# thomasantony/splat

Hardware: AMD Instinct MI355X
Metric: frames_per_sec (higher is better)
Workload: dtype f32

## Files before the change

### splat_amd/csrc/splat_api.hip

```cpp
#include <algorithm>
#include <cmath>
#include <cstdio>
#include <cstdlib>
#include <cstring>
#include <mutex>
#include <new>
#include <string>
#include <unordered_map>
#include <vector>

#include "splat_context.h"

using namespace splat;

static thread_local std::string g_create_error;
static std::mutex g_ledger_mu;
static std::unordered_map<void*, std::pair<splat_ctx*, size_t>> g_ledger;

namespace splat {
CommState** ctx_comm_slot(splat_ctx* c) { return &c->comm; }
hipStream_t ctx_stream(splat_ctx* c) { return c->stream; }
hipStream_t frame_stream(splat_ctx* c) { return (c->last_lane && c->comp2) ? c->comp2 : c->stream; }
int frame_tail(splat_ctx* c) {
    if (c->last_ring < 0 || !c->ring[c->last_ring].used) return SPLAT_OK;
// ... 145 lines not shown

int ensure_lane(splat_ctx* c) {
    if (c->comp2 || c->pipeline == 0) return SPLAT_OK;
    HIP_TRY(c, ensure_copy_stream(c));
    c->comp2 = c->copy_stream;
    return SPLAT_OK;
}

SceneArgs scene_of(const splat_ctx* c) { return {c->n, c->planes, c->orig, c->bounds}; }
HintTable hint_table(const splat_ctx* c, size_t stride) { return {c->need_hint, stride}; }
HintTable hint_table(const splat_ctx* c) { return hint_table(c, c->m_alloc); }

int ensure_bins(splat_ctx* c, unsigned int m) {
    if (m + 1 <= c->m_alloc) return SPLAT_OK;
    int rc = sync_all(c);
    if (rc != SPLAT_OK) return rc;
    c->m_alloc = 0;
    bump_epoch(c);
    c->sort_hint = false;
    dfree(c->zero_layout);
    HIP_TRY(c, dmalloc(c, &c->zero_layout, sizeof(unsigned int) * (size_t)(m + 1)));
    HIP_TRY(c, fill_now(c->zero_layout, 0, sizeof(unsigned int) * (size_t)(m + 1)));
    dfree(c->need_hint);
    HIP_TRY(c, dmalloc(c, &c->need_hint, hint_table(c, (size_t)(m + 1)).bytes()));
    HIP_TRY(c, fill_now(c->need_hint, 0, hint_table(c, (size_t)(m + 1)).bytes()));
    for (Slot& s : c->slots) {
        dfree(s.counts); dfree(s.offsets); dfree(s.cursor); dfree(s.order); dfree(s.lens); dfree(s.counts_b); dfree(s.lay_a); dfree(s.lay_b);
        dfree(s.near_m); dfree(s.redo_layout); dfree(s.redo_cursors); dfree(s.off2);
        s.layout_valid = false; s.flip = 0;
        HIP_TRY(c, dmalloc(c, &s.off2, sizeof(unsigned int) * (size_t)(m + 1)));
        HIP_TRY(c, dmalloc(c, &s.near_m, sizeof(unsigned int) * (size_t)(m + 1)));
        HIP_TRY(c, dmalloc(c, &s.redo_layout, sizeof(unsigned int) * (size_t)(m + 1)));
        HIP_TRY(c, dmalloc(c, &s.redo_cursors, sizeof(unsigned int) * (size_t)(m + 1)));
        HIP_TRY(c, dmalloc(c, &s.counts_b, sizeof(unsigned int) * (size_t)(m + 1)));
        HIP_TRY(c, dmalloc(c, &s.lay_a, sizeof(unsigned int) * (size_t)(m + 1)));
        HIP_TRY(c, dmalloc(c, &s.lay_b, sizeof(unsigned int) * (size_t)(m + 1)));
        HIP_TRY(c, dmalloc(c, &s.lens, sizeof(unsigned int) * (size_t)(m + 1)));
        HIP_TRY(c, dmalloc(c, &s.counts, sizeof(unsigned int) * (size_t)(m + 1)));
        HIP_TRY(c, dmalloc(c, &s.offsets, sizeof(unsigned int) * (size_t)(m + 1)));
        HIP_TRY(c, dmalloc(c, &s.cursor, sizeof(unsigned int) * (size_t)(m + 1)));
        HIP_TRY(c, dmalloc(c, &s.order, sizeof(unsigned int) * (size_t)(m + 1)));
        HIP_TRY(c, fill_now(s.counts, 0, sizeof(unsigned int) * (size_t)(m + 1)));
    }
    c->m_alloc = m + 1;
    return SPLAT_OK;
}
// ... 305 lines not shown
    c->iters_valid = false;
    if (want_iters) {
        if (c->iters_alloc < m * 4u) {
            dfree(c->d_iters); c->iters_alloc = 0;
            HIP_TRY(c, dmalloc(c, &c->d_iters, sizeof(uint2) * (size_t)m * 4u));
            c->iters_alloc = m * 4u;
        }
        HIP_TRY(c, hipMemsetAsync(c->d_iters, 0, sizeof(uint2) * (size_t)m * 4u, cs));
        iters = c->d_iters;
        c->iters_valid = true;
    }
    CompositeArgs comp{};
    comp.s = cs; comp.knobs = &c->knobs; comp.n_tiles = m; comp.fc = c->fc; comp.recs = s.recs; comp.argb = d_argb; comp.status = f.d_st; comp.orig = c->orig;
    comp.fused_sort_max = retained ? 0u : c->fused_sort_max; comp.iters = iters; comp.keep_keys = want_iters || f.retain == SPLAT_RETAIN_WRITER;
    comp.pair_walk = pd.pair_walk != 0;
    comp.libm_exp = (c->cfg.mode & SPLAT_MODE_LIBM_EXP) != 0; comp.clear_first = c->clear_first;
    comp.lists = f.lists; comp.lists.near_m = pd.near_cap ? s.near_m : nullptr;
    comp.keys = f.keys; comp.keys.keys2 = pd.comp_sorts != 0 ? s.keys2 : nullptr;
    if (retained) {
        const bool near = c->ret_set.near_cap != 0u;
        comp.lists.near_m = near ? s.near_m : nullptr; comp.keys.keys2 = near ? s.keys2 : nullptr;
    }
    comp.hints = hint_table(c);
    comp.refine = c->fc.close_width == 0.0f ? pd.refine : 0u;
    launch_composite(comp);
    c->last_near = retained ? c->ret_set.near_cap != 0u : pd.near_cap != 0u;
    HIP_TRY(c, f.mark(6, cs));
    if (want_iters) HIP_TRY(c, hipMemcpyAsync(&c->h_status[f.r], f.d_st, sizeof(FrameStatus), hipMemcpyDeviceToHost, cs));
    HIP_TRY(c, hipEventRecord(f.ev->e[7], cs));
    return SPLAT_OK;
}

int decide_retention(splat_ctx* c, const splat_camera* cam, int* action) {
    splat_retain_input in;
    std::memset(&in, 0, sizeof in);
    static_assert(sizeof(splat_camera) + 2 * sizeof(int32_t) <= sizeof in.cam, "the camera and the slab fit the decision's words");
    std::memcpy(in.cam, cam, sizeof(splat_camera));
    const int32_t slab[2] = {c->slab0, c->slab1};
    std::memcpy(reinterpret_cast<unsigned char*>(in.cam) + sizeof(splat_camera), slab, sizeof slab);
    in.epoch = c->bin_epoch; in.still_frames = c->pol.still_frames;
    in.enabled = (c->retain_lists != 0 && c->knobs.dbg_ntiles == 0u) ? 1 : 0;
    in.overlap = c->overlap; in.one_pass = c->fc.bucket_cap ? 1 : 0;
    splat_retain_decision d;
    const int wr = c->ret_set.ring;
    for (int pass = 0; pass < 2; ++pass) {
        if (c->ret.writer == 1u && wr >= 0) {
// ... 427 lines not shown
        c->env_pinned |= 1u << SPLAT_OPT_NEAR_SELECT_KEYS;
    }
    option_from_env(c, SPLAT_OPT_HOST_ZERO_COPY, "SPLAT_HOST_ZERO_COPY", 0, 1);
    option_from_env(c, SPLAT_OPT_COUNT_FIRST, "SPLAT_COUNT_FIRST", 0, 2);
    if (const char* kg = std::getenv("SPLAT_KEYS_PER_GAUSSIAN")) {
        const int v = std::atoi(kg);
        c->keys_per_gaussian = v <= 0 ? 0u : (unsigned int)std::min(256, std::max(4, v));
        c->env_pinned |= 1u << SPLAT_OPT_KEYS_PER_GAUSSIAN;
    }
    option_from_env(c, SPLAT_OPT_LARGE_SPLAT_TILES, "SPLAT_LARGE_TILES", -1, 1048576);
    option_from_env(c, SPLAT_OPT_LARGE_LIST_MIN, "SPLAT_LARGE_LIST_MIN", -1, 1e9);
    option_from_env(c, SPLAT_OPT_START_REFINE, "SPLAT_START_REFINE", 0, 1);
    option_from_env(c, SPLAT_OPT_RETAIN_LISTS, "SPLAT_RETAIN", 0, 1);
    if (const char* lm = std::getenv("SPLAT_LAYOUT_MOTION")) c->layout_motion = std::atoi(lm) != 0 ? 1 : 0;
    if (const char* k1 = std::getenv("SPLAT_SORT_RADIX_MIN")) c->knobs.sort_radix_min = (unsigned int)std::max(0, std::atoi(k1));
    if (const char* k2 = std::getenv("SPLAT_SCAN_THREADS")) c->knobs.scan_threads = std::atoi(k2);
    if (const char* k3 = std::getenv("SPLAT_DBG_NTILES")) c->knobs.dbg_ntiles = (unsigned int)std::max(0, std::atoi(k3));
    if (const char* k8 = std::getenv("SPLAT_DBG_SELECT_STRIDE")) c->knobs.dbg_select_stride = (unsigned int)std::max(0, std::atoi(k8));
    if (const char* k10 = std::getenv("SPLAT_START_HINTS")) { c->start_hints = std::min(2, std::max(0, std::atoi(k10))); c->env_pinned |= 1u << SPLAT_OPT_START_HINTS; }
    if (const char* k7 = std::getenv("SPLAT_DBG_ONE_PASS_SELECT")) c->one_pass_select = std::atoi(k7) != 0;
    if (const char* k11 = std::getenv("SPLAT_DBG_KEYS2_ENTRIES")) c->knobs.dbg_keys2_entries = std::strtoull(k11, nullptr, 10);
    if (const char* k9 = std::getenv("SPLAT_DBG_HINT_RADIUS")) c->knobs.dbg_hint_radius = std::atoi(k9);
    if (const char* k12 = std::getenv("SPLAT_DBG_SELECT_BLIND")) c->knobs.dbg_select_blind = std::atoi(k12) != 0 ? 1u : 0u;
    if (const char* k5 = std::getenv("SPLAT_DBG_STARTS")) c->knobs.dbg_starts = std::atoi(k5) != 0 ? 1u : 0u;
    if (const char* k4 = std::getenv("SPLAT_COMP_LDS_PAD")) c->knobs.comp_lds_pad = (unsigned int)std::max(0, std::atoi(k4));
    if (const char* k1p = std::getenv("SPLAT_K1_LDS_PAD")) c->knobs.k1_lds_pad = (unsigned int)std::min(48 * 1024, std::max(0, std::atoi(k1p)));
    auto bail = [&](const char* what, hipError_t err) {
        g_create_error = std::string(what) + ": " + hipGetErrorString(err);
        splat_destroy(c);
        return SPLAT_ERR_HIP;
    };
    if ((e = hipSetDevice(cfg->device)) != hipSuccess) return bail("hipSetDevice", e);
    if ((e = init_device_kernels()) != hipSuccess) return bail("hipFuncSetAttribute", e);
    if ((e = hipStreamCreateWithFlags(&c->stream, hipStreamNonBlocking)) != hipSuccess) return bail("hipStreamCreate", e);
    c->own_stream = true;
    {
        int lo = 0, hi = 0;
        (void)hipDeviceGetStreamPriorityRange(&lo, &hi);
        int prio = c->pipeline >= 6 ? (lo + hi) / 2 : hi;
        if (const char* ep = std::getenv("SPLAT_BIN_PRIO")) prio = std::atoi(ep) > 0 ? hi : (std::atoi(ep) < 0 ? lo : (lo + hi) / 2);
        if ((e = hipStreamCreateWithPriority(&c->bin_stream, hipStreamNonBlocking, prio)) != hipSuccess) return bail("hipStreamCreate", e);
        if ((e = hipStreamCreateWithPriority(&c->sort_stream, hipStreamNonBlocking, prio)) != hipSuccess) return bail("hipStreamCreate", e);
    }
    if (c->overlap >= 2 && c->pipeline) { if ((e = ensure_copy_stream(c)) != hipSuccess) return bail("hipStreamCreate", e); c->comp2 = c->copy_stream; }
    for (Slot& s : c->slots) {
        if ((e = dmalloc(c, &s.d_status, sizeof(FrameStatus))) != hipSuccess) return bail("hipMalloc(status)", e);
// ... 1 lines not shown
        if ((e = hipEventCreateWithFlags(&s.ev_ready, hipEventDisableTiming)) != hipSuccess) return bail("hipEventCreate", e);
        if ((e = hipEventCreateWithFlags(&s.ev_binned, hipEventDisableTiming)) != hipSuccess) return bail("hipEventCreate", e);
    }
    if ((e = dmalloc(c, &c->d_status_ring, sizeof(FrameStatus) * EV_RING)) != hipSuccess) return bail("hipMalloc(status ring)", e);
    if ((e = fill_now(c->d_status_ring, 0, sizeof(FrameStatus) * EV_RING)) != hipSuccess) return bail("fill_now(status ring)", e);
    if ((e = hipHostMalloc(&c->h_status, sizeof(FrameStatus) * EV_RING, hipHostMallocCoherent)) != hipSuccess) return bail("hipHostMalloc(status)", e);
    std::memset(c->h_status, 0, sizeof(FrameStatus) * EV_RING);
    for (auto& s : c->ring)
        for (auto& ev : s.e)
            if ((e = hipEventCreate(&ev)) != hipSuccess) return bail("hipEventCreate", e);
    *out = c;
    return SPLAT_OK;
}

void splat_destroy(splat_ctx* c) {
    if (!c) return;
    (void)hipSetDevice(c->cfg.device);
    if (c->bin_stream) (void)hipStreamSynchronize(c->bin_stream);
    if (c->sort_stream) (void)hipStreamSynchronize(c->sort_stream);
    if (c->stream) (void)hipStreamSynchronize(c->stream);
    if (c->copy_stream) (void)hipStreamSynchronize(c->copy_stream);
    if (c->comm) { comm_release(c->comm); c->comm = nullptr; }
    free_scene(c);
    dfree(c->zero_layout); dfree(c->need_hint);
    for (Slot& s : c->slots) {
        dfree(s.counts); dfree(s.offsets); dfree(s.cursor); dfree(s.order); dfree(s.lens); dfree(s.counts_b); dfree(s.lay_a); dfree(s.lay_b);
        dfree(s.near_m); dfree(s.redo_layout); dfree(s.redo_cursors); dfree(s.off2);
        dfree(s.keys); dfree(s.keys2); dfree(s.d_status);
        if (s.ev_ready) (void)hipEventDestroy(s.ev_ready);
        if (s.ev_binned) (void)hipEventDestroy(s.ev_binned);
    }
    dfree(c->d_img); dfree(c->d_iters);
    for (int k = 0; k < splat_ctx::S_IMGS; ++k) {
        dfree(c->s_img[k]);
        if (c->s_rendered[k]) (void)hipEventDestroy(c->s_rendered[k]);
        if (c->s_copied[k]) (void)hipEventDestroy(c->s_copied[k]);
    }
    if (c->copy_stream) { (void)hipStreamSynchronize(c->copy_stream); (void)hipStreamDestroy(c->copy_stream); }
    if (c->h_status) (void)hipHostFree(c->h_status);
    dfree(c->d_status_ring);
    for (auto& s : c->ring)
        for (auto& ev : s.e)
            if (ev) (void)hipEventDestroy(ev);
    if (c->bin_stream) (void)hipStreamDestroy(c->bin_stream);
    if (c->sort_stream) (void)hipStreamDestroy(c->sort_stream);
    if (c->own_stream && c->stream) (void)hipStreamDestroy(c->stream);
    {
// ... 573 lines not shown
```

### splat_amd/csrc/splat_context.h

```cpp
#ifndef SPLAT_CONTEXT_H
#define SPLAT_CONTEXT_H
#include <string>
#include <vector>

#include "splat_internal.h"
#include "../../include/splat_policy.h"
#include "../../include/splat_retain.h"

#define HIP_TRY(ctx, expr)                                                                             \
    do {                                                                                               \
        hipError_t _e = (expr);                                                                        \
        if (_e != hipSuccess) {                                                                        \
            (ctx)->err = std::string(#expr) + ": " + hipGetErrorString(_e);                            \
            return SPLAT_ERR_HIP;                                                                      \
        }                                                                                              \
    } while (0)

namespace splat {
constexpr int N_EV = 9;
constexpr int N_TIMES = 6;
constexpr int EV_RING = 32;
static_assert(EV_RING == SPLAT_POLICY_RING, "the frame policy sees the whole status ring");
constexpr int N_SLOTS = 4;

// ... 88 lines not shown
    uint64_t cap = 0;
    uint64_t cap2 = 0;
    uint64_t keys2_want = 0;
    bool use_buckets = true;
    bool bucket_failed = false;
    uint64_t bucket_bytes = 128ull << 30;
    uint64_t layout_want = 0;
    unsigned int layout_m = 0;
    bool last_one_pass = false;
    unsigned int* zero_layout = nullptr;
    uint64_t dev_bytes = 0, dev_bytes_peak = 0;
    splat::LaunchKnobs knobs;
    float region_spare = 4.0f;
    uint64_t frame_idx = 0;
    uint64_t bin_idx = 0;
    int retain_lists = 1;
    uint64_t bin_epoch = 0;
    splat_retain_state ret{};
    uint64_t frames_retained = 0;
    struct RetainSet {
        int slot = -1, ring = -1;
        unsigned int near_cap = 0;
        splat::FrameStatus status{};
    } ret_set;
    int last_slot = -1;
    bool last_lists_in_memory = false;
    splat::FrameStatus* h_status = nullptr;
    splat::FrameStatus* d_status_ring = nullptr;
    bool clear_first = false;
    uint32_t* d_img = nullptr;
    size_t img_cap = 0;
    static constexpr int S_IMGS = 4;
    uint32_t* s_img[S_IMGS] = {};
    size_t s_cap = 0;
    hipStream_t copy_stream = nullptr;
    hipEvent_t s_rendered[S_IMGS] = {}, s_copied[S_IMGS] = {};
    const uint32_t* s_dst[S_IMGS] = {};
    bool s_used[S_IMGS] = {};
    uint64_t s_idx = 0;
    int s_ring[S_IMGS] = {-1, -1, -1, -1};
    splat_camera s_cam[S_IMGS] = {};
    int slab0 = 0, slab1 = -1;
    splat::EvSet ring[splat::EV_RING];
    int ring_next = 0;
    int last_ring = -1;
    double acc_ms[splat::N_TIMES] = {0, 0, 0, 0, 0, 0};
    uint64_t acc_frames = 0;
// ... 58 lines not shown
```

### splat_amd/csrc/splat_internal.h

```cpp
#ifndef SPLAT_INTERNAL_H
#define SPLAT_INTERNAL_H
#include <hip/hip_runtime.h>
#include <stdint.h>

#include "../../include/splat_hip.h"

#ifndef SPLAT_K1X
#define SPLAT_K1X 0
#endif
#ifndef SPLAT_EXP_STAGE2
#define SPLAT_EXP_STAGE2 0
#endif
#ifndef SPLAT_EXP_K1DUMMY
#define SPLAT_EXP_K1DUMMY 0
#endif
#ifndef SPLAT_EXP_SKIPFULL
#define SPLAT_EXP_SKIPFULL 0
#endif
#ifndef SPLAT_EXP_SORT2
#define SPLAT_EXP_SORT2 0
#endif
#ifndef SPLAT_EXP_K1DROP
#define SPLAT_EXP_K1DROP 0
#endif
// ... 56 lines not shown
    unsigned int n_probe_fail;
    unsigned int pad_;
    unsigned long long n_blocks_culled;
    unsigned long long layout_total;
};

struct Rec {
    float4 a;
    float4 b;
    float4 c;
};

struct LaunchKnobs {
    unsigned int sort_radix_min = 128;
    int scan_threads = 0;
    unsigned int dbg_ntiles = 0;
    unsigned int comp_lds_pad = 0;
    unsigned int k1_lds_pad = 0;
    unsigned int dbg_select_stride = 0;
    unsigned long long dbg_keys2_entries = 0;
    int dbg_hint_radius = -1;
    unsigned int dbg_select_blind = 0;
    unsigned int dbg_starts = 0;
};

struct HintTable {
    unsigned int* base;
    size_t stride;

    static constexpr unsigned int NEED_PLANE = 0u, NEED_PLANES = 4u;
    static constexpr unsigned int DEPTH_PLANE = NEED_PLANE + NEED_PLANES, DEPTH_PLANES = 1u;
    static constexpr unsigned int START_PLANE = DEPTH_PLANE + DEPTH_PLANES, START_PLANES = 4u;
    static constexpr unsigned int REFINE_PLANE = START_PLANE + START_PLANES, REFINE_PLANES = 4u;
    static constexpr unsigned int HINT_WORDS = 13u;
    static_assert(DEPTH_PLANE == 4u && START_PLANE == 5u && REFINE_PLANE == 9u && REFINE_PLANE + REFINE_PLANES == HINT_WORDS,
                  "the four parts tile the table exactly");

    unsigned int* plane(unsigned int k) const { return base ? base + k * stride : nullptr; }
    unsigned int* needs() const { return plane(NEED_PLANE); }
    unsigned int* select_depth() const { return plane(DEPTH_PLANE); }
    unsigned int* starts() const { return plane(START_PLANE); }
    unsigned int* refinement() const { return plane(REFINE_PLANE); }
    size_t words() const { return HINT_WORDS * stride; }
    size_t bytes() const { return sizeof(unsigned int) * words(); }
};

// ... 125 lines not shown
    unsigned int near_cap;
    const unsigned int* need_hint;
    unsigned int* near_thr;
    unsigned int tiles_x, tile_rows;
    unsigned int grid;
    bool at_rest;
    int hint_radius;
};
void launch_select(const SelectArgs& a);

struct CompositeArgs {
    hipStream_t s; const LaunchKnobs* knobs; unsigned int n_tiles; FrameConst fc;
    TileLists lists;
    KeyBuffers keys;
    const Rec* recs; uint32_t* argb; FrameStatus* status; const unsigned int* orig;
    unsigned int fused_sort_max;
    uint2* iters;
    bool keep_keys;
    bool pair_walk;
    bool libm_exp;
    bool clear_first;
    HintTable hints;
    unsigned int refine;
};
void launch_composite(const CompositeArgs& a);
void launch_status_set(hipStream_t s, FrameStatus* status, const FrameStatus& v);
hipError_t init_device_kernels();

struct CommState;
CommState** ctx_comm_slot(splat_ctx* c);
hipStream_t ctx_stream(splat_ctx* c);
hipStream_t frame_stream(splat_ctx* c);
int ctx_device(const splat_ctx* c);
int frame_tail(splat_ctx* c);
int ctx_quiesce(splat_ctx* c);
int ctx_fail(splat_ctx* c, int code, const char* msg);
void comm_release(CommState* s);

}
#endif
```

### splat_amd/csrc/splat_kernels.hip

```cpp
#include <algorithm>
#include <cstddef>
#include <cstdlib>
#include <type_traits>

#include "splat_internal.h"
#include "splat_device_math.h"

namespace splat {
static constexpr unsigned long long KERNELS_EXP2F_TAB[32] = {
    0x3ff0000000000000ull, 0x3fefd9b0d3158574ull, 0x3fefb5586cf9890full, 0x3fef9301d0125b51ull, 0x3fef72b83c7d517bull,
    0x3fef54873168b9aaull, 0x3fef387a6e756238ull, 0x3fef1e9df51fdee1ull, 0x3fef06fe0a31b715ull, 0x3feef1a7373aa9cbull,
    0x3feedea64c123422ull, 0x3feece086061892dull, 0x3feebfdad5362a27ull, 0x3feeb42b569d4f82ull, 0x3feeab07dd485429ull,
    0x3feea47eb03a5585ull, 0x3feea09e667f3bcdull, 0x3fee9f75e8ec5f74ull, 0x3feea11473eb0187ull, 0x3feea589994cce13ull,
    0x3feeace5422aa0dbull, 0x3feeb737b0cdc5e5ull, 0x3feec49182a3f090ull, 0x3feed503b23e255dull, 0x3feee89f995ad3adull,
    0x3feeff76f2fb5e47ull, 0x3fef199bdd85529cull, 0x3fef3720dcef9069ull, 0x3fef5818dcfba487ull, 0x3fef7c97337b9b5full,
    0x3fefa4afa2a490daull, 0x3fefd0765b6e4540ull};
constexpr bool exp2f_tab_is_the_headers() {
    for (int i = 0; i < 32; ++i) if (KERNELS_EXP2F_TAB[i] != EXP2F_TAB_HOST[i]) return false;
    return true;
}
static_assert(exp2f_tab_is_the_headers(), "splat_kernels.hip's copy of EXP2F_TAB differs from splat_device_math.h's");
}


// ... 2254 lines not shown
           (unsigned long long)(unsigned int)__builtin_amdgcn_readfirstlane((int)(unsigned int)v);
}

struct WaveLds { float4 a[64]; float4 b[64]; float4 c[64]; };

#ifndef SPLAT_REFINE_MIN_STEP
#define SPLAT_REFINE_MIN_STEP 8
#endif
#ifndef SPLAT_COMP_WAVES
#define SPLAT_COMP_WAVES 1
#endif
struct CompArgs {
    FrameConst fc;
    const unsigned int* offsets; const unsigned int* order; const unsigned int* lens;
    unsigned long long* keys; const Rec* recs; uint32_t* argb; FrameStatus* status;
    unsigned int fused_sort_max, radix_min;
    uint2* iters;
    unsigned int keep_keys, clear_first;
    const unsigned int* orig;
    unsigned long long* keys2; const unsigned int* near_m;
    unsigned int* need_hint; unsigned int* start_hint; const unsigned int* off2;
    unsigned int* probe_hint;
    unsigned int refine;
};
typedef const __attribute__((address_space(4))) CompArgs* KernArgs;
template <bool PAIR, bool LIBM>
static __device__ void repair_tile(KernArgs ka, unsigned int smem_lds, unsigned int exptab_lds, unsigned int item, bool again);

template <bool PAIR, bool LIBM, int LONGM>
__device__ __forceinline__ void composite_tile(unsigned char* smem, const unsigned long long* exptab, const unsigned int item, const FrameConst& fc,
                                               const unsigned int* __restrict__ offsets, const unsigned int* __restrict__ order,
                                               const unsigned int* __restrict__ lens, unsigned long long* __restrict__ keys,
                                               const Rec* __restrict__ recs, uint32_t* __restrict__ argb,
                                               FrameStatus* __restrict__ status, unsigned int fused_sort_max,
                                               unsigned int radix_min, uint2* __restrict__ iters, unsigned int keep_keys,
                                               const unsigned int* __restrict__ orig, const unsigned int clear_first,
                                               unsigned long long* __restrict__ keys2, const unsigned int* __restrict__ near_m,
                                               unsigned int* __restrict__ need_hint, unsigned int* __restrict__ start_hint,
                                               const unsigned int* __restrict__ off2, KernArgs ka ,
                                               const bool walk_this_wave = true, const bool second_walk = false ) {
    auto late = [&]() -> KernArgs {
        unsigned long long p = (unsigned long long)(size_t)ka;
        asm volatile("" : "+s"(p));
        return (KernArgs)(size_t)p;
    };
    static_assert(sizeof(WaveLds) * 4 <= sort_lds_bytes<256, 2048>(), "staging fits the sort workspace");
    WaveLds* slds = reinterpret_cast<WaveLds*>(smem);
    const unsigned int tile = (unsigned int)__builtin_amdgcn_readfirstlane((int)order[item]);
    const unsigned int tid = threadIdx.x;
    const unsigned int beg = __builtin_amdgcn_readfirstlane(offsets[tile]);
    const unsigned int end = beg + __builtin_amdgcn_readfirstlane(lens[tile]);
    if (beg == end) {
// ... 121 lines not shown
            } else {
                L.a[slot] = r.a; L.b[slot] = r.b;
                L.c[slot] = make_float4(r.c.x, r.c.y, r.c.z, __uint_as_float(base + lane));
            }
        }
        const unsigned int kk = (unsigned int)__builtin_popcountll(m);
        if (pair_layout && (kk & 1u) && lane == 0) {
            float* P = reinterpret_cast<float*>(&L) + (kk >> 1) * 24u + 1u;
            P[0] = 0.0f; P[2] = 0.0f; P[4] = -1.0f; P[6] = -1.0f; P[8] = 0.0f; P[10] = 0.0f; P[12] = 0.0f; P[14] = 0.0f;
            float* Q = reinterpret_cast<float*>(&L) + (kk >> 1) * 24u + 2u;
            Q[16] = 0.0f; Q[17] = 0.0f; Q[20] = 0.0f;
        }
        __builtin_amdgcn_fence(__ATOMIC_ACQUIRE, "wavefront");
        __builtin_amdgcn_wave_barrier();
        return kk;
    };
    auto expv = [&](float x) -> float {
        if constexpr (LIBM) return exp_libm(x, exptab);
        else return exp_neg(x);
    };

    bool need_far = false;
    unsigned int itA = 0, itB = 0;
    float alast = -1.0f;
    if (!need_far) {
        bool found = !inside;
        Rec r;
        unsigned int cntN = min(64u, end - lb), bsN = end - cntN;
        fetch(bsN, cntN, r);
        while (true) {
            const unsigned int bs = bsN, cnt = cntN;
            const unsigned int k = stage(r, cnt, bs, false);
            if (bs > lb) { cntN = min(64u, bs - lb); bsN = bs - cntN; fetch(bsN, cntN, r); }
            unsigned int jsel = 0xffffffffu;
            for (unsigned int j = k; j-- > 0;) {
                const float4 a = L.a[j];
                const bool cov = (fabsf(sxm - a.x) <= a.z) & (fabsf(a.y - sym) <= a.w);
                jsel = (cov & !found) ? j : jsel;
                found = found | cov;
                if (__builtin_amdgcn_ballot_w64(!found) == 0ull) break;
            }
            if (__builtin_amdgcn_ballot_w64(jsel != 0xffffffffu) != 0ull) {
                const unsigned int jr = (jsel != 0xffffffffu) ? jsel : 0u;
                const float4 a = L.a[jr], b = L.b[jr];
                bool cov;
                const float alpha = fragment_alpha(sxm, sym, a, b, expv, cov);
// ... 41 lines not shown
            const unsigned int k = stage(r, cnt, bs, true, true, false, -1, 0u, nA < 32u ? (int)nA : -1);
            nA += nA < 32u ? 1u : 0u;
            if (bs > lb) { cntN = min(64u, bs - lb); bsN = bs - cntN; fetch(bsN, cntN, r); }
            for (unsigned int j = k; j-- > 0;) {
                const float4 a = L.a[j], b = L.b[j];
                const float dx = sxm - a.x, dy = a.y - sym;
                const float p2 = fmaf(dx, fmaf(b.x, dx, b.y * dy), (b.z * dy) * dy) + b.w;
                float alpha = fminf(0.99f, __builtin_amdgcn_exp2f(p2));
                alpha = (p2 < -7.994353f) ? 0.0f : alpha;
                T = fmaf(-alpha, T, T);
                const bool now = !done & (T < fc.early_eps);
                sp = now ? __float_as_uint(a.z) : sp;
                done = done | now;
            }
            itA += k;
            if (__builtin_amdgcn_ballot_w64(!done) == 0ull || bs == lb || bs <= giveup) break;
        }
        unsigned int need = done ? sp : lb;
#pragma unroll
        for (int o = 32; o > 0; o >>= 1) need = min(need, (unsigned int)__shfl_xor((int)need, o));
        ws = (unsigned int)__builtin_amdgcn_readfirstlane((int)need);
        if (ws == 0xffffffffu) ws = end;
    }

    const float cw = fc.close_width;
    float R = (float)((old >> 16) & 0xffu), G = (float)((old >> 8) & 0xffu), B = (float)(old & 0xffu);
    float R2 = 255.0f, G2 = 255.0f, B2 = 255.0f;
    auto shade = [&](auto BRt, const float4& a, const float4& b, const float4& c) {
        constexpr bool BR = decltype(BRt)::value;
        bool cov;
        const float alpha = fragment_alpha(sxm, sym, a, b, expv, cov);
        const float ia = 1.0f - alpha;
        const float ar = alpha * c.x, ag = alpha * c.y, ab = alpha * c.z;
        R = blend_channel(R, ia, ar);
        G = blend_channel(G, ia, ag);
        B = blend_channel(B, ia, ab);
        if (BR) {
            R2 = blend_channel(R2, ia, ar);
            G2 = blend_channel(G2, ia, ag);
            B2 = blend_channel(B2, ia, ab);
        }
    };
    const f2 sxm2 = {sxm, sxm}, sym2 = {sym, sym};
    auto shade_pair = [&](auto BRt, const float4& q0, const float4& q1, const float4& q2, const float4& q3, const float4& q4,
                          const float4& q5) {
        constexpr bool BR = decltype(BRt)::value;
// ... 6 lines not shown
            const float ab = alpha * b;
            f2 s = blend_channel2((f2){R, G}, ia, arg);
            R = s.x; G = s.y;
            B = blend_channel(B, ia, ab);
            if (BR) {
                s = blend_channel2((f2){R2, G2}, ia, arg);
                R2 = s.x; G2 = s.y;
                B2 = blend_channel(B2, ia, ab);
            }
        };
        blend_one(alpha0, (f2){q4.x, q4.y}, q5.x);
        blend_one(alpha1, (f2){q4.z, q4.w}, q5.z);
    };
    auto run = [&](auto BRt, unsigned int start) -> unsigned int {
        constexpr bool BR = decltype(BRt)::value;
        Rec r;
        unsigned int kb = start < end ? (end - 1u - start) >> 6 : 0u;
        unsigned int bsN = start, cntN = start < end ? (end - (kb << 6)) - start : 0u;
        if (cntN) fetch(bsN, cntN, r);
        while (cntN) {
            const unsigned int bs = bsN, cnt = cntN;
            const bool reuse = kb < nA;
            const unsigned int abase = (end - lb >= ((kb + 1u) << 6)) ? end - ((kb + 1u) << 6) : lb;
            const unsigned int k = stage(r, cnt, bs, true, false, PAIR, reuse ? (int)kb : -1, bs - abase);
            bsN = bs + cnt; cntN = min(64u, end - bsN); kb -= cntN ? 1u : 0u;
            if (cntN) fetch(bsN, cntN, r);
            if constexpr (PAIR) {
                const float4* P4 = reinterpret_cast<const float4*>(&L);
                for (unsigned int j = 0; j < (k + 1u) / 2u; ++j)
                    shade_pair(BRt, P4[6 * j], P4[6 * j + 1], P4[6 * j + 2], P4[6 * j + 3], P4[6 * j + 4], P4[6 * j + 5]);
            } else {
                for (unsigned int j = 0; j < k; ++j) shade(BRt, L.a[j], L.b[j], L.c[j]);
            }
            itB += k;
            if (BR && __builtin_amdgcn_ballot_w64(inside & ((R2 - R > cw) | (G2 - G > cw) | (B2 - B > cw))) == 0ull) return bsN;
        }
        return end;
    };
    unsigned int start = ws;
    while (!need_far) {
        if (start <= lb) {
            if (has_far) { need_far = true; break; }
            R = (float)((old >> 16) & 0xffu); G = (float)((old >> 8) & 0xffu); B = (float)(old & 0xffu);
            run(std::false_type{}, lb);
            break;
        }
        R = G = B = 0.0f; R2 = G2 = B2 = 255.0f;
// ... 20 lines not shown
    uint2* const iters_l = kl->iters;
    if (iters_l != nullptr && lane == 0) {
        const unsigned int kk = kl->keep_keys;
        uint2 v = (kk & 2u) ? make_uint2(end - beg, end - max(start, beg)) : make_uint2(itA, itB);
        if (second_walk && !(kk & 2u)) { const uint2 o = iters_l[item * 4u + wave]; v.x += o.x; v.y += o.y; }
        iters_l[item * 4u + wave] = v;
    }
    if constexpr (LONGM != 0) {
        unsigned int* const need_l = kl->need_hint;
        if (need_l != nullptr && end - beg > 2048u && lane == 0u) need_l[tile * 4u + wave] = need_far ? 0xffffffffu : end - max(start, lb);
    }
    unsigned int* const start_l = kl->start_hint;
    if (start_l != nullptr && early && !need_far && (scanned || start != ws) && lane == 0u) {
        unsigned int used = max(end - max(start, lb), 1u);
        if (!has_far && used > (end - beg) - ((end - beg) >> 2)) used = end - beg;
        start_l[tile * 4u + wave] = used;
    }
    if (probe != 0u && lane == 0u) {
        const bool failed = (probe >> 31) != 0u;
        const unsigned int half = (probe & 0xffffu) >> 1;
        const unsigned int step = failed ? (half >= (unsigned int)SPLAT_REFINE_MIN_STEP ? half : 0u) : probe;
        if (!failed) start_l[tile * 4u + wave] = end - ws;
        kl->probe_hint[tile * 4u + wave] = (kl->refine & 0xffff0000u) | step;
    }
    if (need_far) return true;
    if (inside)
        kl->argb[(size_t)py * kl->fc.W + px] = ((uint32_t)A << 24) | ((uint32_t)R << 16) | ((uint32_t)G << 8) | (uint32_t)B;
    return false;
    };
    if constexpr (LONGM != 2) {
        (void)walk_list();
    } else {
        const bool again = walk_list();
        if (has_far && __syncthreads_or(again ? 1 : 0) != 0) {
            if (tid == 0u) atomicAdd(&late()->status->n_near_fallback, 1u);
            repair_tile<PAIR, LIBM>(ka, (unsigned int)(size_t)(__attribute__((address_space(3))) unsigned char*)smem,
                                    (unsigned int)(size_t)(__attribute__((address_space(3))) const unsigned long long*)exptab, item, again);
        }
    }
}

template <bool PAIR, bool LIBM>
static __device__ __attribute__((noinline)) void repair_tile(KernArgs ka, unsigned int smem_lds, unsigned int exptab_lds, unsigned int item, bool again) {
    const unsigned long long kp = uniform_u64((unsigned long long)(size_t)ka);
    const KernArgs k = (KernArgs)(size_t)kp;
    unsigned char* const smem = (unsigned char*)(__attribute__((address_space(3))) unsigned char*)(size_t)__builtin_amdgcn_readfirstlane((int)smem_lds);
    const unsigned long long* const exptab = (const unsigned long long*)(__attribute__((address_space(3))) const unsigned long long*)(size_t)__builtin_amdgcn_readfirstlane((int)exptab_lds);
    const unsigned int it = (unsigned int)__builtin_amdgcn_readfirstlane((int)item);
    FrameConst fc;
    {
        const __attribute__((address_space(4))) unsigned int* src = (const __attribute__((address_space(4))) unsigned int*)&k->fc;
        unsigned int* dst = reinterpret_cast<unsigned int*>(&fc);
#pragma unroll
        for (unsigned int q = 0; q < sizeof(FrameConst) / 4u; ++q) dst[q] = src[q];
    }
    composite_tile<PAIR, LIBM, 1>(smem, exptab, it, fc, k->offsets, k->order, k->lens, k->keys, k->recs, k->argb, k->status, k->fused_sort_max, k->radix_min,
                                  k->iters, k->keep_keys, k->orig, k->clear_first, k->keys2, nullptr, k->need_hint, k->start_hint, k->off2, k, again, true);
    if (threadIdx.x == 0u) {
        const unsigned int tile = k->order[it];
        const_cast<unsigned int*>(k->near_m)[tile] = k->lens[tile];
    }
}

__global__ __launch_bounds__(256) void select_near_kernel(const unsigned int* __restrict__ offsets, const unsigned int* __restrict__ order,
                                                          const unsigned int* __restrict__ lens, unsigned long long* __restrict__ keys,
                                                          unsigned long long* __restrict__ keys2, FrameStatus* __restrict__ status,
                                                          const unsigned int* __restrict__ orig, unsigned int radix_min, unsigned int near_cap,
                                                          const unsigned int* __restrict__ need_hint, unsigned int* __restrict__ near_m,
                                                          unsigned int tiles_x, unsigned int tile_rows, unsigned int* __restrict__ near_thr,
                                                          unsigned int n_slots, unsigned int at_rest, const unsigned int* __restrict__ off2,
                                                          int hint_radius, unsigned int blind) {
    __shared__ __attribute__((aligned(16))) unsigned char smem[sort_lds_bytes<256, 2048>()];
    if (status->overflow) return;
  for (unsigned int slot = blockIdx.x; slot < n_slots; slot += gridDim.x) {
    const unsigned int tile = (unsigned int)__builtin_amdgcn_readfirstlane((int)order[slot]);
    const unsigned int n = (unsigned int)__builtin_amdgcn_readfirstlane((int)lens[tile]);
    if (n < 2048u) return;
    if (n == 2048u) continue;
    const unsigned int beg = (unsigned int)__builtin_amdgcn_readfirstlane((int)offsets[tile]);
    unsigned long long* const k2 = keys2 + (unsigned int)__builtin_amdgcn_readfirstlane((int)off2[tile]);
    unsigned int want = near_cap, deepest, thr = 0u;
    {
        unsigned int* const word = reinterpret_cast<unsigned int*>(smem);
// ... 62 lines not shown
    }
    __syncthreads();
  }
}

__global__ void status_set_kernel(FrameStatus* __restrict__ status, const FrameStatus v) { *status = v; }
void launch_status_set(hipStream_t s, FrameStatus* status, const FrameStatus& v) {
    hipLaunchKernelGGL(status_set_kernel, dim3(1), dim3(1), 0, s, status, v);
}

template <bool PAIR, bool LIBM, int LONGM>
__global__ __launch_bounds__(256, (LONGM != 0 && !PAIR) ? 7 : SPLAT_COMP_WAVES) __attribute__((amdgpu_num_sgpr(96))) void composite_exact_kernel(CompArgs a) {
    __shared__ __attribute__((aligned(16))) unsigned char smem[sort_lds_bytes<256, 2048>()];
    __shared__ unsigned long long exptab[LIBM ? 32 : 1];
    if (a.status->overflow) return;
    if constexpr (LIBM) {
        static_assert(!PAIR, "the libm exponential is built for the one-record walk only");
        if (threadIdx.x < 32) exptab[threadIdx.x] = EXP2F_TAB[threadIdx.x];
        __syncthreads();
    }
    composite_tile<PAIR, LIBM, LONGM>(smem, exptab, blockIdx.x, a.fc, a.offsets, a.order, a.lens, a.keys, a.recs, a.argb, a.status, a.fused_sort_max, a.radix_min, a.iters, a.keep_keys, a.orig,
                                      a.clear_first, a.keys2, a.near_m, a.need_hint, a.start_hint, a.off2, (KernArgs)__builtin_amdgcn_kernarg_segment_ptr());
}

static inline unsigned int blocks_for(uint64_t n, unsigned int bs) { return (unsigned int)((n + bs - 1) / bs); }

hipError_t init_device_kernels() {
    hipError_t e = hipFuncSetAttribute(reinterpret_cast<const void*>(sort_tiles_kernel<1024, 16384>),
                                       hipFuncAttributeMaxDynamicSharedMemorySize, sort_lds_bytes<1024, 16384>());
    if (e != hipSuccess) return e;
    return hipFuncSetAttribute(reinterpret_cast<const void*>(sort_tiles_kernel<512, 8192>),
                               hipFuncAttributeMaxDynamicSharedMemorySize, sort_lds_bytes<512, 8192>());
}

void launch_pack_scene(hipStream_t s, uint64_t n, const float* pos4, const float* cov3d, const float* opacity,
                       const float* sh, const unsigned int* perm, float4* planes) {
    if (!n) return;
    hipLaunchKernelGGL(pack_scene_kernel, dim3(blocks_for(n, 256)), dim3(256), 0, s, n, pos4, cov3d, opacity, sh, perm, planes);
}
void launch_cov3d(hipStream_t s, uint64_t n, const float* scales3, const float* rot4, float* cov3d) {
    if (!n) return;
    hipLaunchKernelGGL(cov3d_kernel, dim3(blocks_for(n, 256)), dim3(256), 0, s, n, scales3, rot4, cov3d);
}
static inline unsigned int sort_groups(uint64_t n) { return (unsigned int)((n + SORT_TILE - 1) / SORT_TILE); }
static inline unsigned int box_groups(uint64_t n) { return std::min(blocks_for(n, 256), BOX_GROUPS_MAX); }
size_t scene_order_small_bytes(uint64_t n) {
// ... 136 lines not shown
    if (a.knobs->dbg_hint_radius >= 0) hint_radius = a.knobs->dbg_hint_radius;
    if (a.knobs->dbg_select_stride) grid = (n_tiles + a.knobs->dbg_select_stride - 1u) / a.knobs->dbg_select_stride;
    if (!grid) grid = (n_tiles + 7u) / 8u;
    hipLaunchKernelGGL(select_near_kernel, dim3(std::min(grid, n_tiles)), dim3(256), 0, a.s, a.lists.offsets, a.lists.order, a.lists.lens, a.keys.keys, a.keys.keys2, a.status, a.orig, a.knobs->sort_radix_min,
                       std::min(std::max(a.near_cap, 64u), 2048u), a.need_hint, a.lists.near_m, a.tiles_x, a.tile_rows, a.near_thr, n_tiles, a.at_rest ? 1u : 0u, off2, std::min(std::max(hint_radius, 0), 7), a.knobs->dbg_select_blind);
}
void launch_composite(const CompositeArgs& c) {
    unsigned int n_tiles = c.n_tiles;
    if (!n_tiles) return;
    const unsigned int* off2 = c.lists.off2;
    if (!off2) off2 = c.lists.offsets;
    if (c.knobs->dbg_ntiles) n_tiles = std::min(n_tiles, c.knobs->dbg_ntiles);
    const unsigned int pad = c.knobs->comp_lds_pad;
    unsigned long long* keys2 = c.keys.keys2;
    const unsigned int* near_m = c.lists.near_m;
    unsigned int *need_hint = c.hints.needs(), *start_hint = c.hints.starts(), *probe_hint = c.hints.refinement();
    const bool near = near_m != nullptr && keys2 != nullptr && need_hint != nullptr;
    const unsigned int flags = (c.keep_keys ? 1u : 0u) | (c.knobs->dbg_starts ? 2u : 0u);
    CompArgs a;
    a.fc = c.fc; a.offsets = c.lists.offsets; a.order = c.lists.order; a.lens = c.lists.lens; a.keys = c.keys.keys; a.recs = c.recs; a.argb = c.argb; a.status = c.status;
    a.fused_sort_max = c.fused_sort_max; a.radix_min = c.knobs->sort_radix_min; a.iters = c.iters; a.keep_keys = flags; a.clear_first = c.clear_first ? 1u : 0u;
    a.orig = c.orig; a.keys2 = keys2; a.near_m = near_m; a.need_hint = near ? need_hint : nullptr; a.start_hint = start_hint; a.off2 = off2;
    a.probe_hint = probe_hint; a.refine = (probe_hint != nullptr && start_hint != nullptr) ? c.refine : 0u;
    auto go = [&](auto kern) { hipLaunchKernelGGL(kern, dim3(n_tiles), dim3(256), pad, c.s, a); };
    if (near) {
        if (c.libm_exp) go(composite_exact_kernel<false, true, 2>);
        else if (c.pair_walk) go(composite_exact_kernel<true, false, 2>);
        else go(composite_exact_kernel<false, false, 2>);
    } else if (keys2 != nullptr) {
        if (c.libm_exp) go(composite_exact_kernel<false, true, 1>);
        else if (c.pair_walk) go(composite_exact_kernel<true, false, 1>);
        else go(composite_exact_kernel<false, false, 1>);
    } else {
        if (c.libm_exp) go(composite_exact_kernel<false, true, 0>);
        else if (c.pair_walk) go(composite_exact_kernel<true, false, 0>);
        else go(composite_exact_kernel<false, false, 0>);
    }
}

}
```

Baseline: 4825.

## Cache per-wave staging visibility masks across retained frames in composite

Adds a per-wave cache of staging masks (stage_nv count plus 32 mask words per wave) that retained frames reuse, so composite can skip recomputing the culling verdicts for staged batches. A writer frame resets the cache, and a new retained composite kernel variant reads and extends it. It costs extra device buffers, global loads and stores per wave, and adds a correctness risk if the cached verdicts go stale. The feature is on by default through dbg_stage_cache=1.

```diff
diff --git a/splat_amd/csrc/splat_api.hip b/splat_amd/csrc/splat_api.hip
--- a/splat_amd/csrc/splat_api.hip
+++ b/splat_amd/csrc/splat_api.hip
@@ -191,6 +191,7 @@
     HIP_TRY(c, dmalloc(c, &c->zero_layout, sizeof(unsigned int) * (size_t)(m + 1)));
     HIP_TRY(c, fill_now(c->zero_layout, 0, sizeof(unsigned int) * (size_t)(m + 1)));
     dfree(c->need_hint);
+    dfree(c->stage_nv); dfree(c->stage_mask);
     HIP_TRY(c, dmalloc(c, &c->need_hint, hint_table(c, (size_t)(m + 1)).bytes()));
     HIP_TRY(c, fill_now(c->need_hint, 0, hint_table(c, (size_t)(m + 1)).bytes()));
     for (Slot& s : c->slots) {
@@ -542,6 +543,22 @@
         comp.lists.near_m = near ? s.near_m : nullptr; comp.keys.keys2 = near ? s.keys2 : nullptr;
     }
     comp.hints = hint_table(c);
+    if (c->knobs.dbg_stage_cache != 0u && f.retain == SPLAT_RETAIN_WRITER) {
+        const size_t waves = (size_t)c->m_alloc * 4u;
+        if (!c->stage_nv || !c->stage_mask) {
+            dfree(c->stage_nv); dfree(c->stage_mask);
+            HIP_TRY(c, dmalloc(c, &c->stage_nv, sizeof(unsigned int) * waves));
+            HIP_TRY(c, dmalloc(c, &c->stage_mask, sizeof(unsigned long long) * 32u * waves));
+        }
+        HIP_TRY(c, hipMemsetAsync(c->stage_nv, 0, sizeof(unsigned int) * waves, cs));
+        c->ret_set.frames = 0;
+    }
+    if (retained && c->knobs.dbg_stage_cache != 0u && c->stage_nv && c->stage_mask) {
+        comp.stage_nv = c->stage_nv; comp.stage_mask = c->stage_mask;
+        if (c->knobs.dbg_stage_cache == 2u && c->ret_set.frames >= 2u)
+            HIP_TRY(c, hipMemsetAsync(c->stage_mask, 0, sizeof(unsigned long long) * 32u * (size_t)c->m_alloc * 4u, cs));
+        c->ret_set.frames++;
+    }
     comp.refine = c->fc.close_width == 0.0f ? pd.refine : 0u;
     launch_composite(comp);
     c->last_near = retained ? c->ret_set.near_cap != 0u : pd.near_cap != 0u;
@@ -1015,6 +1032,7 @@
     if (const char* k11 = std::getenv("SPLAT_DBG_KEYS2_ENTRIES")) c->knobs.dbg_keys2_entries = std::strtoull(k11, nullptr, 10);
     if (const char* k9 = std::getenv("SPLAT_DBG_HINT_RADIUS")) c->knobs.dbg_hint_radius = std::atoi(k9);
     if (const char* k12 = std::getenv("SPLAT_DBG_SELECT_BLIND")) c->knobs.dbg_select_blind = std::atoi(k12) != 0 ? 1u : 0u;
+    if (const char* k13 = std::getenv("SPLAT_DBG_STAGE_CACHE")) c->knobs.dbg_stage_cache = (unsigned int)std::min(2, std::max(0, std::atoi(k13)));
     if (const char* k5 = std::getenv("SPLAT_DBG_STARTS")) c->knobs.dbg_starts = std::atoi(k5) != 0 ? 1u : 0u;
     if (const char* k4 = std::getenv("SPLAT_COMP_LDS_PAD")) c->knobs.comp_lds_pad = (unsigned int)std::max(0, std::atoi(k4));
     if (const char* k1p = std::getenv("SPLAT_K1_LDS_PAD")) c->knobs.k1_lds_pad = (unsigned int)std::min(48 * 1024, std::max(0, std::atoi(k1p)));
@@ -1062,7 +1080,7 @@
     if (c->copy_stream) (void)hipStreamSynchronize(c->copy_stream);
     if (c->comm) { comm_release(c->comm); c->comm = nullptr; }
     free_scene(c);
-    dfree(c->zero_layout); dfree(c->need_hint);
+    dfree(c->zero_layout); dfree(c->need_hint); dfree(c->stage_nv); dfree(c->stage_mask);
     for (Slot& s : c->slots) {
         dfree(s.counts); dfree(s.offsets); dfree(s.cursor); dfree(s.order); dfree(s.lens); dfree(s.counts_b); dfree(s.lay_a); dfree(s.lay_b);
         dfree(s.near_m); dfree(s.redo_layout); dfree(s.redo_cursors); dfree(s.off2);
diff --git a/splat_amd/csrc/splat_context.h b/splat_amd/csrc/splat_context.h
--- a/splat_amd/csrc/splat_context.h
+++ b/splat_amd/csrc/splat_context.h
@@ -134,7 +134,10 @@
         int slot = -1, ring = -1;
         unsigned int near_cap = 0;
         splat::FrameStatus status{};
+        unsigned int frames = 0;
     } ret_set;
+    unsigned int* stage_nv = nullptr;
+    unsigned long long* stage_mask = nullptr;
     int last_slot = -1;
     bool last_lists_in_memory = false;
     splat::FrameStatus* h_status = nullptr;
diff --git a/splat_amd/csrc/splat_internal.h b/splat_amd/csrc/splat_internal.h
--- a/splat_amd/csrc/splat_internal.h
+++ b/splat_amd/csrc/splat_internal.h
@@ -102,6 +102,7 @@
     int dbg_hint_radius = -1;
     unsigned int dbg_select_blind = 0;
     unsigned int dbg_starts = 0;
+    unsigned int dbg_stage_cache = 1;
 };
 
 struct HintTable {
@@ -273,6 +274,8 @@
     bool clear_first;
     HintTable hints;
     unsigned int refine;
+    unsigned int* stage_nv;
+    unsigned long long* stage_mask;
 };
 void launch_composite(const CompositeArgs& a);
 void launch_status_set(hipStream_t s, FrameStatus* status, const FrameStatus& v);
diff --git a/splat_amd/csrc/splat_kernels.hip b/splat_amd/csrc/splat_kernels.hip
--- a/splat_amd/csrc/splat_kernels.hip
+++ b/splat_amd/csrc/splat_kernels.hip
@@ -2300,12 +2300,13 @@
     unsigned int* need_hint; unsigned int* start_hint; const unsigned int* off2;
     unsigned int* probe_hint;
     unsigned int refine;
+    unsigned int* stage_nv; unsigned long long* stage_mask;
 };
 typedef const __attribute__((address_space(4))) CompArgs* KernArgs;
-template <bool PAIR, bool LIBM>
+template <bool PAIR, bool LIBM, bool KEEP>
 static __device__ void repair_tile(KernArgs ka, unsigned int smem_lds, unsigned int exptab_lds, unsigned int item, bool again);
 
-template <bool PAIR, bool LIBM, int LONGM>
+template <bool PAIR, bool LIBM, int LONGM, bool KEEP = false>
 __device__ __forceinline__ void composite_tile(unsigned char* smem, const unsigned long long* exptab, const unsigned int item, const FrameConst& fc,
                                                const unsigned int* __restrict__ offsets, const unsigned int* __restrict__ order,
                                                const unsigned int* __restrict__ lens, unsigned long long* __restrict__ keys,
@@ -2473,6 +2474,20 @@
 
     bool need_far = false;
     unsigned int itA = 0, itB = 0;
+    unsigned int nvc = 0xffffffffu;
+    if constexpr (KEEP) {
+        if (!second_walk) {
+            const KernArgs kc = late();
+            const unsigned int* const nv_l = kc->stage_nv;
+            const unsigned long long kept = kc->stage_mask[(size_t)(tile * 4u + wave) * 32u + (lane & 31u)];
+            nvc = min((unsigned int)__builtin_amdgcn_readfirstlane((int)nv_l[tile * 4u + wave]), 32u);
+            __builtin_amdgcn_fence(__ATOMIC_RELEASE, "wavefront");
+            __builtin_amdgcn_wave_barrier();
+            if (lane < nvc) wmask[lane] = kept;
+            __builtin_amdgcn_fence(__ATOMIC_ACQUIRE, "wavefront");
+            __builtin_amdgcn_wave_barrier();
+        }
+    }
     float alast = -1.0f;
     if (!need_far) {
         bool found = !inside;
@@ -2560,6 +2575,8 @@
         ws = (unsigned int)__builtin_amdgcn_readfirstlane((int)need);
         if (ws == 0xffffffffu) ws = end;
     }
+    const bool keeping = KEEP && nvc != 0xffffffffu && !scanned;
+    if (keeping) nA = nvc;
 
     const float cw = fc.close_width;
     float R = (float)((old >> 16) & 0xffu), G = (float)((old >> 8) & 0xffu), B = (float)(old & 0xffu);
@@ -2612,7 +2629,8 @@
             const unsigned int bs = bsN, cnt = cntN;
             const bool reuse = kb < nA;
             const unsigned int abase = (end - lb >= ((kb + 1u) << 6)) ? end - ((kb + 1u) << 6) : lb;
-            const unsigned int k = stage(r, cnt, bs, true, false, PAIR, reuse ? (int)kb : -1, bs - abase);
+            const bool keep = KEEP && keeping && !reuse && kb < 32u && bs == abase;
+            const unsigned int k = stage(r, cnt, bs, true, false, PAIR, reuse ? (int)kb : -1, bs - abase, keep ? (int)kb : -1);
             bsN = bs + cnt; cntN = min(64u, end - bsN); kb -= cntN ? 1u : 0u;
             if (cntN) fetch(bsN, cntN, r);
             if constexpr (PAIR) {
@@ -2679,6 +2697,21 @@
         const unsigned int step = failed ? (half >= (unsigned int)SPLAT_REFINE_MIN_STEP ? half : 0u) : probe;
         if (!failed) start_l[tile * 4u + wave] = end - ws;
         kl->probe_hint[tile * 4u + wave] = (kl->refine & 0xffff0000u) | step;
+    }
+    if (KEEP && keeping && !need_far && max(start, lb) < end) {
+        const unsigned int s = max(start, lb), kf = (end - 1u - s) >> 6;
+        const unsigned int ab = (end - lb >= ((kf + 1u) << 6)) ? end - ((kf + 1u) << 6) : lb;
+        const unsigned int nv_new = min(kf + (s == ab ? 1u : 0u), 32u);
+        unsigned int* const nv_l = kl->stage_nv;
+        const unsigned int nv_old = (unsigned int)__builtin_amdgcn_readfirstlane((int)nv_l[tile * 4u + wave]);
+        if (nv_new > nv_old) {
+            __builtin_amdgcn_fence(__ATOMIC_RELEASE, "wavefront");
+            __builtin_amdgcn_wave_barrier();
+            if (lane >= nv_old && lane < nv_new) kl->stage_mask[(size_t)(tile * 4u + wave) * 32u + lane] = wmask[lane];
+            if (lane == 0u) nv_l[tile * 4u + wave] = nv_new;
+            __builtin_amdgcn_fence(__ATOMIC_ACQUIRE, "wavefront");
+            __builtin_amdgcn_wave_barrier();
+        }
     }
     if (need_far) return true;
     if (inside)
@@ -2691,13 +2724,13 @@
         const bool again = walk_list();
         if (has_far && __syncthreads_or(again ? 1 : 0) != 0) {
             if (tid == 0u) atomicAdd(&late()->status->n_near_fallback, 1u);
-            repair_tile<PAIR, LIBM>(ka, (unsigned int)(size_t)(__attribute__((address_space(3))) unsigned char*)smem,
+            repair_tile<PAIR, LIBM, KEEP>(ka, (unsigned int)(size_t)(__attribute__((address_space(3))) unsigned char*)smem,
                                     (unsigned int)(size_t)(__attribute__((address_space(3))) const unsigned long long*)exptab, item, again);
         }
     }
 }
 
-template <bool PAIR, bool LIBM>
+template <bool PAIR, bool LIBM, bool KEEP>
 static __device__ __attribute__((noinline)) void repair_tile(KernArgs ka, unsigned int smem_lds, unsigned int exptab_lds, unsigned int item, bool again) {
     const unsigned long long kp = uniform_u64((unsigned long long)(size_t)ka);
     const KernArgs k = (KernArgs)(size_t)kp;
@@ -2716,6 +2749,8 @@
     if (threadIdx.x == 0u) {
         const unsigned int tile = k->order[it];
         const_cast<unsigned int*>(k->near_m)[tile] = k->lens[tile];
+        unsigned int* const nv_l = KEEP ? k->stage_nv : nullptr;
+        if (nv_l != nullptr) { nv_l[tile * 4u + 0u] = 0u; nv_l[tile * 4u + 1u] = 0u; nv_l[tile * 4u + 2u] = 0u; nv_l[tile * 4u + 3u] = 0u; }
     }
 }
 
@@ -2824,6 +2859,19 @@
     composite_tile<PAIR, LIBM, LONGM>(smem, exptab, blockIdx.x, a.fc, a.offsets, a.order, a.lens, a.keys, a.recs, a.argb, a.status, a.fused_sort_max, a.radix_min, a.iters, a.keep_keys, a.orig,
                                       a.clear_first, a.keys2, a.near_m, a.need_hint, a.start_hint, a.off2, (KernArgs)__builtin_amdgcn_kernarg_segment_ptr());
 }
+template <bool PAIR, bool LIBM, int LONGM>
+__global__ __launch_bounds__(256, (LONGM != 0 && !PAIR) ? 7 : SPLAT_COMP_WAVES) __attribute__((amdgpu_num_sgpr(96))) void composite_retained_kernel(CompArgs a) {
+    static_assert(LONGM == 0 || LONGM == 2, "a retained frame's long lists are in order in their regions, or selections");
+    __shared__ __attribute__((aligned(16))) unsigned char smem[sort_lds_bytes<256, 2048>()];
+    __shared__ unsigned long long exptab[LIBM ? 32 : 1];
+    if (a.status->overflow) return;
+    if constexpr (LIBM) {
+        if (threadIdx.x < 32) exptab[threadIdx.x] = EXP2F_TAB[threadIdx.x];
+        __syncthreads();
+    }
+    composite_tile<PAIR, LIBM, LONGM, true>(smem, exptab, blockIdx.x, a.fc, a.offsets, a.order, a.lens, a.keys, a.recs, a.argb, a.status, a.fused_sort_max, a.radix_min, a.iters, a.keep_keys, a.orig,
+                                            a.clear_first, a.keys2, a.near_m, a.need_hint, a.start_hint, a.off2, (KernArgs)__builtin_amdgcn_kernarg_segment_ptr());
+}
 
 static inline unsigned int blocks_for(uint64_t n, unsigned int bs) { return (unsigned int)((n + bs - 1) / bs); }
 
@@ -3006,8 +3054,18 @@
     a.fused_sort_max = c.fused_sort_max; a.radix_min = c.knobs->sort_radix_min; a.iters = c.iters; a.keep_keys = flags; a.clear_first = c.clear_first ? 1u : 0u;
     a.orig = c.orig; a.keys2 = keys2; a.near_m = near_m; a.need_hint = near ? need_hint : nullptr; a.start_hint = start_hint; a.off2 = off2;
     a.probe_hint = probe_hint; a.refine = (probe_hint != nullptr && start_hint != nullptr) ? c.refine : 0u;
+    const bool keep_verdicts = c.stage_nv != nullptr && c.stage_mask != nullptr && (near || keys2 == nullptr);
+    a.stage_nv = keep_verdicts ? c.stage_nv : nullptr; a.stage_mask = keep_verdicts ? c.stage_mask : nullptr;
     auto go = [&](auto kern) { hipLaunchKernelGGL(kern, dim3(n_tiles), dim3(256), pad, c.s, a); };
-    if (near) {
+    if (keep_verdicts && near) {
+        if (c.libm_exp) go(composite_retained_kernel<false, true, 2>);
+        else if (c.pair_walk) go(composite_retained_kernel<true, false, 2>);
+        else go(composite_retained_kernel<false, false, 2>);
+    } else if (keep_verdicts) {
+        if (c.libm_exp) go(composite_retained_kernel<false, true, 0>);
+        else if (c.pair_walk) go(composite_retained_kernel<true, false, 0>);
+        else go(composite_retained_kernel<false, false, 0>);
+    } else if (near) {
         if (c.libm_exp) go(composite_exact_kernel<false, true, 2>);
         else if (c.pair_walk) go(composite_exact_kernel<true, false, 2>);
         else go(composite_exact_kernel<false, false, 2>);
```

Result: faster. 4977, median of 6 (+3.2%).
